# bentotten/radiation_ppo

Hardware: AMD Instinct MI355X
Metric: env steps/sec (whole node) at 4096 envs; PPO iters/sec at 1/2/4/8 GPUs (higher is better)
Workload: dtype f32 policy / f64+int32 env

## Files before the change

include/radsearch.h:

```cpp
#ifndef RADSEARCH_H
#define RADSEARCH_H

#include <stddef.h>
#include <stdint.h>

#ifdef __cplusplus
extern "C" {
#endif

#define RS_ABI_VERSION 4
#define RS_OBS_DIM 11
#define RS_NUM_ACTIONS 9
#define RS_MAX_AGENTS 8
#define RS_MAX_OBS 7

typedef void* rs_stream_t;
typedef struct rs_handle rs_handle;

enum {
    RS_OK = 0,
    RS_ERR_INVALID_ARG = 1,
    RS_ERR_HIP = 2,
    RS_ERR_WORKSPACE = 3,
    RS_ERR_UNSUPPORTED = 4
// ... 37 lines not shown
int rs_create(const rs_config* cfg, void* workspace, size_t workspace_bytes, rs_stream_t stream, rs_handle** out);
void rs_destroy(rs_handle* h);

int rs_state_field(rs_handle* h, const char* name, void** dev_ptr, int32_t* elem_bytes, int32_t* rows, int32_t* cols);

int rs_set_epoch_end(rs_handle* h, rs_stream_t stream);

int rs_reset(rs_handle* h, const uint8_t* mask, float* obs, float* reward, float* team, uint8_t* done,
             const rs_info* info, rs_stream_t stream);

int rs_refresh(rs_handle* h, const uint8_t* mask, const int32_t* src_xy, const int32_t* det_xy, const int32_t* intensity,
               const int32_t* bkg, const int32_t* num_obs, const int32_t* rects, float* obs, float* reward, float* team,
               uint8_t* done, const rs_info* info, rs_stream_t stream);

int rs_step(rs_handle* h, const int8_t* actions, float* obs, float* reward, float* team, uint8_t* done,
            const rs_info* info, rs_stream_t stream);

int rs_action_uniforms(rs_handle* h, float* u, rs_stream_t stream);

int rs_error_flags(rs_handle* h, rs_stream_t stream, uint32_t* flags_out);

int rs_gae(const float* rew, const float* val, const uint8_t* cut, const float* last_val, float* adv, float* ret,
           int32_t T, int32_t M, double gamma, double lam, rs_stream_t stream);

typedef struct rs_mlp_params {
    const float *w1, *b1, *w2, *b2, *w3, *b3;
} rs_mlp_params;

int rs_policy_forward(const rs_mlp_params* actor, const rs_mlp_params* critic, const float* x, int32_t M,
                      float* logits, float* value, rs_stream_t stream);

typedef struct rs_rollout_args {
    int32_t steps_per_epoch;
    int32_t steps_per_episode;
    float* obs;
    int64_t* act;
    float* logp;
    float* val;
    float* rew;
    float* last_val;
    uint8_t* cut;
    float* source_tar;
    float* cur_obs;
    double* w_count;
    double* w_mean;
    double* w_sq;
// ... 223 lines not shown
```

radiation_ppo_amd/_lib.py:

```python
import ctypes as C
import os

import torch

_PKG = os.path.dirname(os.path.abspath(__file__))
LIB_PATH = os.environ.get("RS_LIB_PATH") or os.path.join(_PKG, "lib", "librs_hip.so")

RS_OBS_DIM = 11
RS_MAX_AGENTS = 8
RS_MAX_OBS = 7

ENVERR_ZERO_DIST = 1
ENVERR_IDLE_STALL = 2
ENVERR_CORRECT_CAP = 4
ENVERR_BAD_ACTION = 8
ENVERR_NO_PATH = 16


class RsConfig(C.Structure):
    _fields_ = [
        ("num_envs", C.c_int32), ("num_agents", C.c_int32), ("obstruction_count", C.c_int32),
        ("enforce_grid_boundaries", C.c_int32), ("bbox", C.c_int32 * 4), ("observation_area", C.c_int32 * 2),
        ("falloff", C.c_int32), ("geom_group_size", C.c_int32), ("seed", C.c_uint32), ("env_id_base", C.c_uint32),
        ("coord_noise", C.c_int32), ("debug_spawn", C.c_int32),
# ... 53 lines not shown
                              C.c_void_p, C.c_void_p, C.c_void_p]),
    ("rs_adam_step", C.c_int, [C.POINTER(RsMlpParams), C.POINTER(RsMlpParams), C.c_void_p, C.c_void_p, C.c_void_p, C.c_void_p,
                               C.c_void_p, C.c_float, C.c_float, C.c_void_p]),
    ("rs_ppo_update_step", C.c_int, [C.POINTER(RsMlpParams), C.POINTER(RsMlpParams), C.POINTER(RsPpoBatch), C.c_void_p, C.c_void_p,
                                     C.c_void_p, C.c_void_p, C.c_void_p, C.c_void_p, C.c_float, C.c_float, C.c_void_p]),
    ("rs_maps_state_bytes", C.c_size_t, [C.c_int32, C.c_int32, C.c_int32, C.c_int32, C.c_int32]),
    ("rs_maps_create", C.c_int, [C.c_int32, C.c_int32, C.c_int32, C.c_int32, C.c_int32, C.c_double, C.c_void_p, C.c_void_p,
                                 C.c_size_t, C.c_void_p, C.POINTER(C.c_void_p)]),
    ("rs_maps_destroy", None, [C.c_void_p]),
    ("rs_maps_reset", C.c_int, [C.c_void_p, C.c_void_p, C.c_void_p]),
    ("rs_maps_update", C.c_int, [C.c_void_p, C.c_void_p, C.c_void_p, C.c_void_p, C.c_void_p, C.c_void_p]),
    ("rs_maps_stack", C.c_int, [C.c_void_p, C.c_void_p, C.c_void_p, C.c_void_p]),
    ("rs_maps_field", C.c_int, [C.c_void_p, C.c_char_p, C.POINTER(C.c_void_p), C.POINTER(C.c_int32), C.POINTER(C.c_int32),
                                C.POINTER(C.c_int32)]),
    ("rs_cnn_trunk_slab_row", C.c_int32, [C.c_int32]),
    ("rs_cnn_trunk_slab_rows", C.c_int32, [C.c_int64, C.c_int32]),
    ("rs_cnn_trunk_scratch_floats", C.c_int32, [C.c_int32]),
    ("rs_cnn_trunk_forward", C.c_int, [C.c_void_p, C.c_void_p, C.c_void_p, C.c_int32, C.c_int32, C.c_int64, C.c_void_p, C.c_void_p,
                                       C.c_void_p, C.c_void_p, C.c_void_p, C.c_void_p, C.c_void_p, C.c_void_p, C.c_void_p, C.c_void_p]),
    ("rs_cnn_trunk_backward", C.c_int, [C.c_void_p, C.c_void_p, C.c_void_p, C.c_int32, C.c_int32, C.c_int64, C.c_void_p, C.c_void_p,
                                        C.c_void_p, C.c_void_p, C.c_void_p, C.c_void_p, C.c_void_p, C.c_void_p]),
    ("rs_gae", C.c_int, [C.c_void_p, C.c_void_p, C.c_void_p, C.c_void_p, C.c_void_p, C.c_void_p, C.c_int32,
                         C.c_int32, C.c_double, C.c_double, C.c_void_p]),
    ("rs_pfgru_step", C.c_int, [C.c_void_p, C.c_void_p, C.c_void_p, C.c_void_p, C.c_void_p, C.c_void_p, C.c_void_p, C.c_void_p,
                                C.c_int32, C.c_double, C.c_void_p, C.c_int32, C.c_int32, C.c_void_p]),
    ("rs_pfgru_step_recorded", C.c_int, [C.c_void_p] * 7 + [C.c_int32, C.c_double, C.c_void_p, C.c_int32, C.c_int32, C.c_void_p]),
    ("rs_pfgru_pass", C.c_int, [C.c_void_p] * 7 + [C.c_double, C.c_void_p, C.c_void_p, C.c_int32, C.c_int32, C.c_void_p]),
    ("rs_pfgru_reset", C.c_int, [C.c_void_p, C.c_void_p, C.c_void_p, C.c_void_p, C.c_void_p, C.c_void_p, C.c_int32, C.c_int32,
                                 C.c_void_p]),
    ("rs_pfgru_sized_weight_floats", C.c_int32, [C.c_int32]),
    ("rs_pfgru_sized_step", C.c_int, [C.c_void_p] * 8 + [C.c_int32, C.c_double, C.c_void_p, C.c_int32, C.c_int32, C.c_int32, C.c_void_p]),
    ("rs_pfgru_sized_pass", C.c_int, [C.c_void_p] * 7 + [C.c_double, C.c_void_p, C.c_void_p, C.c_int32, C.c_int32, C.c_int32, C.c_void_p]),
    ("rs_pfgru_sized_step_recorded", C.c_int, [C.c_void_p] * 7 + [C.c_int32, C.c_double, C.c_void_p, C.c_int32, C.c_int32, C.c_int32,
                                                                    C.c_void_p]),
    ("rs_pfgru_sized_reset", C.c_int, [C.c_void_p] * 6 + [C.c_int32, C.c_int32, C.c_int32, C.c_void_p]),
    ("rs_pfgru_draws", C.c_int, [C.c_void_p, C.c_int32, C.c_int32, C.c_void_p, C.c_void_p, C.c_void_p, C.c_void_p]),
    ("rs_pfgru_train", C.c_int, [C.c_void_p] * 15 + [C.c_int32, C.c_int32, C.c_double, C.c_double, C.c_double, C.c_double, C.c_void_p]),
    ("rs_pfgru_train_keyed", C.c_int, [C.c_void_p] * 14 + [C.c_int32, C.c_int32, C.c_double, C.c_double, C.c_double, C.c_double, C.c_void_p]),
    ("rs_pfgru_sized_train_weight_floats", C.c_int32, [C.c_int32]),
    ("rs_pfgru_sized_train_grad_floats", C.c_int32, [C.c_int32]),
    ("rs_pfgru_sized_draws", C.c_int, [C.c_void_p, C.c_int32, C.c_int32, C.c_int32, C.c_void_p, C.c_void_p, C.c_void_p, C.c_void_p]),
    ("rs_pfgru_sized_train", C.c_int, [C.c_void_p] * 15 + [C.c_int32, C.c_int32, C.c_double, C.c_double, C.c_double, C.c_double, C.c_int32,
                                       C.c_void_p]),
    ("rs_rnn_policy_step", C.c_int, [C.c_void_p] * 10 + [C.c_int32, C.c_void_p]),
    ("rs_rnn_policy_step_rows", C.c_int, [C.c_void_p, C.c_void_p, C.c_int32, C.c_void_p, C.c_int32, C.c_void_p, C.c_void_p, C.c_int32, C.c_void_p,
                                          C.c_void_p, C.c_void_p, C.c_void_p, C.c_void_p, C.c_int32, C.c_void_p, C.c_int32, C.c_void_p]),
# ... 84 lines not shown
```

radiation_ppo_amd/csrc/rs_env.hip:

```cpp
#include <hip/hip_runtime.h>
#include <stdint.h>
#include <stdlib.h>
#include <string.h>
#include <new>

#include "../../include/radsearch.h"
#include "rs_device.hpp"
#include "rs_handle.hpp"

template <bool HAS_OBS>
__global__ void __launch_bounds__(64, (HAS_OBS ? 4 : 1)) rs_step_kernel(RsParams P, const int8_t* __restrict__ actions, float* obs, RsOut O) {
    extern __shared__ __align__(16) unsigned char smem[];
    int* lds_geo = reinterpret_cast<int*>(smem);
    float* tile = reinterpret_cast<float*>(smem + (HAS_OBS ? RS_MAX_VERT * RS_WAVE * 4 : 0));
    int* flags = reinterpret_cast<int*>(tile + RS_WAVE * rs_tile_stride(P.A));
    const int lane = threadIdx.x & 63;
    const int n = blockIdx.x * blockDim.x + threadIdx.x;
    const bool active = n < P.N;
    RsGeo g{lds_geo, 0, 0, 0};
    if (HAS_OBS) rs_load_geo(P, n, active, lds_geo, g);
    flags[lane] = active ? 1 : 0;
    __syncthreads();
    if (active) {
        RsOut o = O;
// ... 204 lines not shown
            const int t = tb - u;
            if (t >= t_lo) {
                const double r = (double)r8[u], v = (double)v8[u];
                if (c8[u]) {
                    const double lv = (double)l8[u];
                    v_next = lv;
                    r_acc = lv;
                    a_acc = 0.0;
                }
                const double delta = r + gamma * v_next - v;
                a_acc = delta + gl * a_acc;
                r_acc = r + gamma * r_acc;
                if (t <= t_hi) {
                    const size_t i = (size_t)t * M + m;
                    adv[i] = (float)a_acc;
                    ret[i] = (float)r_acc;
                }
                v_next = v;
            }
        }
#pragma unroll
        for (int u = 0; u < RS_GAE_U; ++u) { r8[u] = rn[u]; v8[u] = vn[u]; l8[u] = ln[u]; c8[u] = cn[u]; }
    }
}

static inline size_t align_up(size_t x, size_t a) { return (x + a - 1) / a * a; }

struct Carver {
    unsigned char* base; size_t off; rs_handle* h;
    template <typename T> T* take(const char* name, int rows, int cols) {
        off = align_up(off, 256);
        T* p = base ? reinterpret_cast<T*>(base + off) : nullptr;
        if (h) { h->fields[h->n_fields++] = rs_field{name, (void*)p, (int)sizeof(T), rows, cols}; }
        off += sizeof(T) * (size_t)rows * (size_t)cols;
        return p;
    }
};

static bool cfg_ok(const rs_config* c) {
    if (!c) return false;
    if (c->num_envs < 1 || c->num_agents < 1 || c->num_agents > RS_MAX_AGENTS) return false;
    if (c->obstruction_count < -1 || c->obstruction_count > RS_MAX_OBS) return false;
    if (c->geom_group_size < 1) return false;
    if (c->bbox[2] <= c->bbox[0] || c->bbox[3] <= c->bbox[1]) return false;
    if (c->bbox[2] > 16000 || c->bbox[3] > 16000 || c->bbox[0] < -16000 || c->bbox[1] < -16000) return false;
    if (c->observation_area[0] < 0 || c->observation_area[1] <= c->observation_area[0]) return false;
// ... 179 lines not shown
        hipStreamSynchronize(s) != hipSuccess) rc = RS_ERR_HIP;
    uint32_t acc = 0;
    if (rc == RS_OK) for (int i = 0; i < N; ++i) acc |= host[i];
    delete[] host;
    *flags_out = acc;
    return rc;
}

int rs_gae(const float* rew, const float* val, const uint8_t* cut, const float* last_val, float* adv, float* ret,
           int32_t T, int32_t M, double gamma, double lam, rs_stream_t stream) {
    if (!rew || !val || !cut || !last_val || !adv || !ret || T < 1 || M < 1) return RS_ERR_INVALID_ARG;
    hipStream_t s = static_cast<hipStream_t>(stream);
    const int col_waves = (M + 63) / 64;
    int chunks = (512 + col_waves - 1) / col_waves;
    chunks = chunks < 1 ? 1 : (chunks > 16 ? 16 : chunks);
    int chunk = (T + chunks - 1) / chunks;
    if (chunk < 32) chunk = 32;
    chunks = (T + chunk - 1) / chunk;
    hipLaunchKernelGGL(rs_gae_kernel, dim3(col_waves, chunks), dim3(64), 0, s, rew, val, cut, last_val, adv, ret, T, M,
                       gamma, gamma * lam, chunk);
    return hipGetLastError() == hipSuccess ? RS_OK : RS_ERR_HIP;
}

#ifdef RS_STEP_STAMPS
int rs_debug_step_stamps(unsigned long long* out, int clear) {
    if (hipDeviceSynchronize() != hipSuccess) return RS_ERR_HIP;
    if (out && hipMemcpyFromSymbol(out, HIP_SYMBOL(rs_step_stamp_table), sizeof(unsigned long long) * 16) != hipSuccess) return RS_ERR_HIP;
    if (clear) {
        unsigned long long z[16] = {0};
        if (hipMemcpyToSymbol(HIP_SYMBOL(rs_step_stamp_table), z, sizeof(z)) != hipSuccess) return RS_ERR_HIP;
    }
    return RS_OK;
}
#endif

}
```

radiation_ppo_amd/csrc/rs_ppo.hip:

```cpp
#include <hip/hip_runtime.h>
#include <stdint.h>
#include <stdlib.h>
#include <string.h>

#include "../../include/radsearch.h"
#include "rs_mlp.hpp"
#include "rs_handle.hpp"

static inline RsMlpParams to_dev(const rs_mlp_params* p) { return RsMlpParams{p->w1, p->b1, p->w2, p->b2, p->w3, p->b3}; }

__device__ __forceinline__ void rs_exchange_x(const float (&xo)[RS_IN_PAD], float (&xp)[RS_IN_PAD]) {
#pragma unroll
    for (int k = 0; k < RS_IN_PAD; ++k) xp[k] = __shfl_xor(xo[k], 32);
}

__global__ void __launch_bounds__(64) rs_policy_forward_kernel(RsMlpParams pa, RsMlpParams pc, const float* __restrict__ x, int M,
                                                               float* __restrict__ logits, float* __restrict__ value) {
    extern __shared__ __align__(16) float smem_f[];
    RsMlpLds<8> A; RsMlpLds<1> Cn;
    A.carve(smem_f);
    Cn.carve(smem_f + rs_mlp_lds_floats(8));
    A.fill(pa); Cn.fill(pc);
    __syncthreads();
    const int lane = threadIdx.x & 63;
// ... 260 lines not shown
    if (!actor || !critic || !grads || !m || !v || !state) return RS_ERR_INVALID_ARG;
    const RsParamSeg S = rs_param_seg(actor, critic);
    const int o = S.off[12];
    hipStream_t s = static_cast<hipStream_t>(stream);
    hipLaunchKernelGGL(rs_adam_apply_kernel, dim3((o + 255) / 256), dim3(256), 0, s, S, grads, m, v, stats, state, lr, kl_threshold);
    hipLaunchKernelGGL(rs_adam_commit_kernel, dim3(1), dim3(1), 0, s, stats, grads + o, state, kl_threshold);
    return hipGetLastError() == hipSuccess ? RS_OK : RS_ERR_HIP;
}

struct RsGradWs { float *pa, *pc; double *sa, *sc; int* snap; };

static RsGradWs rs_grad_ws(void* workspace) {
    const int slabs = RS_GRAD_BLOCKS;
    RsGradWs w;
    w.pa = static_cast<float*>(workspace);
    w.pc = w.pa + (size_t)slabs * rs_net_params(8);
    w.sa = reinterpret_cast<double*>((reinterpret_cast<uintptr_t>(w.pc + (size_t)slabs * rs_net_params(1)) + 255) & ~uintptr_t(255));
    w.sc = w.sa + (size_t)slabs * 5;
    w.snap = reinterpret_cast<int*>(w.sc + (size_t)slabs * 5);
    return w;
}

static int rs_launch_k7(const rs_mlp_params* actor, const rs_mlp_params* critic, const rs_ppo_batch* batch, const RsGradWs& w,
                        const int32_t* stop_flag, const rs_update_state* ust, hipStream_t s) {
    const size_t lds_a = sizeof(float) * (size_t)rs_grad2_lds_floats(8);
    const size_t lds_c = sizeof(float) * (size_t)rs_grad2_lds_floats(1);
    if (hipFuncSetAttribute(reinterpret_cast<const void*>(rs_ppo_grad2_kernel<8>), hipFuncAttributeMaxDynamicSharedMemorySize, (int)lds_a) != hipSuccess ||
        hipFuncSetAttribute(reinterpret_cast<const void*>(rs_ppo_grad2_kernel<1>), hipFuncAttributeMaxDynamicSharedMemorySize, (int)lds_c) != hipSuccess)
        return RS_ERR_HIP;
    int threads = 512;
#ifdef RS_K7_STAMPS
    if (const char* e = getenv("RS_K7_THREADS")) threads = atoi(e) == 256 ? 256 : 512;
#endif
    hipLaunchKernelGGL(rs_ppo_grad2_kernel<8>, dim3(RS_GRAD_BLOCKS), dim3(threads), lds_a, s, to_dev(actor), *batch, w.pa, w.sa, stop_flag,
                       (const rs_update_state*)nullptr, (int*)nullptr);
    hipLaunchKernelGGL(rs_ppo_grad2_kernel<1>, dim3(RS_GRAD_BLOCKS), dim3(threads), lds_c, s, to_dev(critic), *batch, w.pc, w.sc, stop_flag,
                       ust, ust ? w.snap : (int*)nullptr);
    return RS_OK;
}

int rs_ppo_grad(const rs_mlp_params* actor, const rs_mlp_params* critic, const rs_ppo_batch* batch, float* grads,
                double* stats, void* workspace, const int32_t* stop_flag, rs_stream_t stream) {
    if (!actor || !critic || !batch || !grads || !stats || !workspace || batch->M < 1) return RS_ERR_INVALID_ARG;
    if (reinterpret_cast<uintptr_t>(workspace) & 255u) return RS_ERR_WORKSPACE;
    hipStream_t s = static_cast<hipStream_t>(stream);
    const RsGradWs w = rs_grad_ws(workspace);
    if (const int rc = rs_launch_k7(actor, critic, batch, w, stop_flag, nullptr, s)) return rc;
    const int np = rs_net_params(8) + rs_net_params(1);
    hipLaunchKernelGGL(rs_ppo_reduce_kernel, dim3((np + 63) / 64), dim3(1024), 0, s, w.pa, w.pc, w.sa, w.sc, RS_GRAD_BLOCKS, grads, stats,
                       batch->alpha, batch->vf_coef, stop_flag);
    return hipGetLastError() == hipSuccess ? RS_OK : RS_ERR_HIP;
}

int rs_ppo_update_step(const rs_mlp_params* actor, const rs_mlp_params* critic, const rs_ppo_batch* batch, float* grads,
                       double* stats, void* workspace, float* m, float* v, rs_update_state* state, float lr, float kl_threshold,
                       rs_stream_t stream) {
    if (!actor || !critic || !batch || !grads || !stats || !workspace || !m || !v || !state || batch->M < 1) return RS_ERR_INVALID_ARG;
    if (reinterpret_cast<uintptr_t>(workspace) & 255u) return RS_ERR_WORKSPACE;
    hipStream_t s = static_cast<hipStream_t>(stream);
    const RsGradWs w = rs_grad_ws(workspace);
    if (const int rc = rs_launch_k7(actor, critic, batch, w, &state->stopped, state, s)) return rc;
    const int np = rs_net_params(8) + rs_net_params(1);
    hipLaunchKernelGGL(rs_ppo_tail_kernel, dim3((np + 63) / 64), dim3(1024), 0, s, w.pa, w.pc, w.sa, w.sc, RS_GRAD_BLOCKS, grads, stats,
                       batch->alpha, batch->vf_coef, rs_param_seg(actor, critic), m, v, state, w.snap, lr, kl_threshold);
    return hipGetLastError() == hipSuccess ? RS_OK : RS_ERR_HIP;
}

#ifdef RS_K7_STAMPS
int rs_debug_k7_stamps(unsigned long long* out, int clear) {
    if (hipDeviceSynchronize() != hipSuccess) return RS_ERR_HIP;
    if (out && hipMemcpyFromSymbol(out, HIP_SYMBOL(rs_k7_stamp_table), sizeof(unsigned long long) * 2 * RS_K7_NPH) != hipSuccess) return RS_ERR_HIP;
    if (clear) {
        unsigned long long z[2 * RS_K7_NPH] = {0};
        if (hipMemcpyToSymbol(HIP_SYMBOL(rs_k7_stamp_table), z, sizeof(z)) != hipSuccess) return RS_ERR_HIP;
    }
    return RS_OK;
}
#endif

int rs_policy_forward(const rs_mlp_params* actor, const rs_mlp_params* critic, const float* x, int32_t M,
                      float* logits, float* value, rs_stream_t stream) {
    if (!actor || !critic || !x || M < 1) return RS_ERR_INVALID_ARG;
    const int groups = (M + 63) / 64;
    const int grid = groups < 2048 ? groups : 2048;
// ... 8 lines not shown
```

radiation_ppo_amd/csrc/rs_ppo_grad2.hpp:

```cpp
#pragma once
#include "rs_mlp.hpp"

#define RS_T2 33

#ifdef RS_K7_STAMPS
#define RS_K7_NPH 16
__device__ unsigned long long rs_k7_stamp_table[2][RS_K7_NPH];
#define RS_STAMP_ENTRY const unsigned long long st_rt0 = __builtin_amdgcn_s_memrealtime(); const unsigned long long st_t0 = rs_k7_now();
#define RS_STAMP_DECL unsigned long long st_acc[RS_K7_NPH] = {0}; unsigned long long st_last = rs_k7_now(); st_acc[12] = st_last - st_t0;
#define RS_STAMP_EXIT(net) do { RS_STAMP(13); if ((threadIdx.x & 63) == 0) { st_acc[14] = __builtin_amdgcn_s_memrealtime() - st_rt0; \
                           for (int q = 0; q < RS_K7_NPH; ++q) atomicAdd(&rs_k7_stamp_table[net][q], st_acc[q]); } } while (0)
#define RS_STAMP(i) do { __builtin_amdgcn_sched_barrier(0); asm volatile("; RS_STAMP_MARK " #i); const unsigned long long t_ = rs_k7_now(); st_acc[i] += t_ - st_last; st_last = t_; \
                         __builtin_amdgcn_sched_barrier(0); } while (0)
__device__ __forceinline__ unsigned long long rs_k7_now() {
    unsigned long long t;
    asm volatile("s_memtime %0\n\ts_waitcnt lgkmcnt(0)" : "=s"(t) :: "memory");
    return t;
}
#else
#define RS_STAMP_ENTRY
#define RS_STAMP_DECL
#define RS_STAMP_EXIT(net)
#ifdef RS_K7_NO_PHASE_FENCE
#define RS_STAMP(i) do {} while (0)
#else
#define RS_STAMP(i) __builtin_amdgcn_sched_barrier(0)
#endif
#endif
#define RS_XRAW 400
#define RS_XSC 192
#define RS_G2_WAVE_FLOATS ((64 + 32) * RS_T2 + RS_XRAW + RS_XSC + 64)

__host__ __device__ constexpr int rs_grad2_lds_floats(int nout) {
    return ((rs_mlp_lds_floats(nout) + 3) & ~3) + 2 * 2 * 16 * 64 + 2 * 4 * 64 + 8 * RS_G2_WAVE_FLOATS;
}

__device__ __forceinline__ float rs_other_half(float x, int h) {
    const auto r = __builtin_amdgcn_permlane32_swap(__float_as_uint(x), __float_as_uint(x), false, false);
    return __uint_as_float(h ? r[0] : r[1]);
}

__device__ __forceinline__ void rs_stage32(float* T, const f32x16& v, int c, int h) {
#pragma unroll
    for (int r = 0; r < 16; ++r) T[rs_kappa(r, h) * RS_T2 + c] = v[r];
}

template <int NOUT>
__global__ void __launch_bounds__(512, 2) rs_ppo_grad2_kernel(RsMlpParams prm, rs_ppo_batch B, float* __restrict__ partial,
                                                              double* __restrict__ stat_partial, const int* __restrict__ stop,
                                                              const rs_update_state* __restrict__ ust, int* __restrict__ snap) {
    extern __shared__ __align__(16) float smem_f[];
    if (snap && blockIdx.x == 0 && threadIdx.x == 0) { snap[0] = ust->adam_step; snap[1] = ust->stopped; }
    if (stop && *stop) return;
    RS_STAMP_ENTRY
    RsMlpLds<NOUT> W;
    W.carve(smem_f);
    float* w2tf = smem_f + ((rs_mlp_lds_floats(NOUT) + 3) & ~3);
    float* w3tf = w2tf + 2 * 2 * 16 * 64;
    const int wid = __builtin_amdgcn_readfirstlane(threadIdx.x >> 6);
    const int lane = threadIdx.x & 63, h = lane >> 5, c = lane & 31;
    const int l15 = lane & 15, l4 = lane >> 4;
    float* Qt = w3tf + 2 * 4 * 64 + wid * RS_G2_WAVE_FLOATS;
    float* Pt = Qt + 64 * RS_T2;
    float* xraw = Pt + 32 * RS_T2;
    float* xsc = xraw + RS_XRAW;
    float* dbl = xsc + RS_XSC;
    float* w1b = W.w1f;
    for (int i = threadIdx.x; i < 2 * 6 * 64; i += blockDim.x) {
        const int l = i & 63, s = (i >> 6) % 6, it = i / (6 * 64);
        const int row = 32 * it + (l & 31), k = 2 * s + (l >> 5);
        w1b[i] = RS_TANH_PRESCALE * ((k < RS_IN) ? prm.w1[row * RS_IN + k] : prm.b1[row]);
    }
    for (int i = threadIdx.x; i < 2 * 2 * 16 * 64; i += blockDim.x) {
        const int ri = i & 3, l = (i >> 2) & 63, r4 = (i >> 8) & 3, kt = (i >> 10) & 1, it = i >> 11;
        const int r = 4 * r4 + ri;
        w2tf[i] = prm.w2[(32 * kt + rs_kappa(r, l >> 5)) * RS_HID + 32 * it + (l & 31)];
        W.w2f[i] = RS_TANH_PRESCALE * prm.w2[(32 * it + (l & 31)) * RS_HID + 32 * kt + rs_kappa(r, l >> 5)];
    }
    for (int i = threadIdx.x; i < 2 * 4 * 64; i += blockDim.x) {
        int l = i & 63, sq = (i >> 6) & 3, it = i >> 8;
        int o = 2 * sq + (l >> 5);
        w3tf[i] = (o < NOUT) ? prm.w3[o * RS_HID + 32 * it + (l & 31)] : 0.0f;
    }
    for (int i = threadIdx.x; i < 2 * NOUT * 32; i += blockDim.x) {
        const int q = i & 31, o = (i >> 5) % NOUT, hh = i / (32 * NOUT);
        W.w3h[i] = prm.w3[o * RS_HID + 32 * (q >> 4) + rs_kappa(q & 15, hh)];
    }
    for (int i = threadIdx.x; i < 64; i += blockDim.x) W.b2[i] = RS_TANH_PRESCALE * prm.b2[i];
    for (int i = threadIdx.x; i < NOUT; i += blockDim.x) W.b3[i] = prm.b3[i];
    dbl[lane] = 0.0f;
    __syncthreads();

    const int M = B.M;
    const int groups = (M + 31) / 32;
    const int wave_g = blockIdx.x * 8 + wid, n_waves = gridDim.x * 8;

    f32x16 acc2[2][2];
    f32x4 acc1[4], acc3[4];
#pragma unroll
    for (int a = 0; a < 2; ++a)
#pragma unroll
        for (int r = 0; r < 16; ++r) { acc2[a][0][r] = 0.f; acc2[a][1][r] = 0.f; }
#pragma unroll
    for (int a = 0; a < 4; ++a)
#pragma unroll
        for (int r = 0; r < 4; ++r) { acc1[a][r] = 0.f; acc3[a][r] = 0.f; }
    f32x4 accs;
#pragma unroll
    for (int r = 0; r < 4; ++r) accs[r] = 0.f;

    const int trips = (groups + n_waves - 1) / n_waves;
    const long x_last = (long)M * RS_IN - 1;
    auto dma_rows = [&](int g) {
        const char* gx = reinterpret_cast<const char*>(B.x + (long)g * (32 * RS_IN));
        const int lim = (int)(x_last - (long)g * (32 * RS_IN));
#pragma unroll
        for (int i = 0; i < 6; ++i) {
            const int o = min(i * 64 + lane, lim);
// ... 342 lines not shown
            for (int s = 0; s < 8; ++s) {
                float a0_n = 0.f, a1_n = 0.f;
                if (s + 1 < 8) {
                    a0_n = Pt[l15 * RS_T2 + 4 * (s + 1) + l4];
                    a1_n = Pt[(16 + l15) * RS_T2 + 4 * (s + 1) + l4];
                }
                acc1[2 * it + 0] = __builtin_amdgcn_mfma_f32_16x16x4f32(a0_c, xb[s], acc1[2 * it + 0], 0, 0, 0);
                acc1[2 * it + 1] = __builtin_amdgcn_mfma_f32_16x16x4f32(a1_c, xb[s], acc1[2 * it + 1], 0, 0, 0);
                a0_c = a0_n; a1_c = a1_n;
            }
        }
        rs_wave_sync();
        RS_STAMP(11);
    }
    constexpr int RS_REST = rs_net_params(NOUT) - 64 * 64;
    static_assert(8 * 64 * 64 <= rs_grad2_lds_floats(NOUT) && 8 * ((RS_REST + 1) & ~1) + 2 * 8 * 5 <= rs_grad2_lds_floats(NOUT),
                  "the epilogue's slabs must fit K7's LDS");
    int tid_e = threadIdx.x;
    asm volatile("" : "+v"(tid_e));
    const int lane_e = tid_e & 63, h_e = lane_e >> 5, c_e = lane_e & 31, l15_e = lane_e & 15, l4_e = lane_e >> 4;
    asm volatile("s_waitcnt vmcnt(0)" ::: "memory");
    const float db2v = dbl[lane_e];
    __syncthreads();
    float* outp = partial + (size_t)blockIdx.x * rs_net_params(NOUT);
    {
        float* g_w2 = smem_f + wid * (64 * 64);
#pragma unroll
        for (int it = 0; it < 2; ++it)
#pragma unroll
            for (int r = 0; r < 16; ++r) {
                const int row = 32 * it + rs_kappa(r, h_e);
                g_w2[row * 64 + c_e] = acc2[it][0][r];
                g_w2[row * 64 + 32 + c_e] = acc2[it][1][r];
            }
    }
    __syncthreads();
    for (int i = tid_e; i < 64 * 64; i += blockDim.x) {
        float v = 0.0f + smem_f[i];
#pragma unroll
        for (int wv = 1; wv < 8; ++wv) v += smem_f[wv * (64 * 64) + i];
        outp[64 * RS_IN + 64 + i] = v;
    }
    float db3r[NOUT];
#pragma unroll
    for (int o = 0; o < NOUT; ++o) db3r[o] = __shfl(accs[o & 3], 16 * (o >> 2));
    double sv[5];
    {
// ... 15 lines not shown
                if (l15_e < RS_IN) g_w1[row * RS_IN + l15_e] = acc1[u][q];
                if (l15_e == RS_IN) g_b1[row] = acc1[u][q];
                const int o = 4 * l4_e + q;
                if (o < NOUT) g_w3[o * 64 + 16 * u + l15_e] = acc3[u][q];
            }
        if (lane_e == 0) {
#pragma unroll
            for (int o = 0; o < NOUT; ++o) g_b3[o] = db3r[o];
#pragma unroll
            for (int q = 0; q < 5; ++q) sred[wid * 5 + q] = sv[q];
        }
    }
    __syncthreads();
    for (int i = tid_e; i < RS_REST; i += blockDim.x) {
        float v = 0.0f + smem_f[i];
#pragma unroll
        for (int wv = 1; wv < 8; ++wv) v += smem_f[wv * RS_RSTR + i];
        outp[i < 64 * RS_IN + 64 ? i : i + 64 * 64] = v;
    }
    if (tid_e < 5) {
        double v = 0.0 + sred[tid_e];
#pragma unroll
        for (int wv = 1; wv < 8; ++wv) v += sred[wv * 5 + tid_e];
        stat_partial[(size_t)blockIdx.x * 5 + tid_e] = v;
    }
    RS_STAMP_EXIT(NOUT == 8 ? 0 : 1);
}
```

radiation_ppo_amd/ppo.py:

```python
import ctypes as C
import os
from dataclasses import dataclass
from typing import Any, Dict, List, Optional

import torch
import torch.distributed as dist
import torch.nn as nn

from . import _lib
from .envs import RadSearchVec, gae as rs_gae_call


class FFActorCritic(nn.Module):

    def __init__(self, state_dim: int = 11, action_dim: int = 8, hidden: int = 64):
        super().__init__()
        self.actor = nn.Sequential(nn.Linear(state_dim, hidden), nn.Tanh(), nn.Linear(hidden, hidden), nn.Tanh(),
                                   nn.Linear(hidden, action_dim), nn.Softmax(dim=-1))
        self.critic = nn.Sequential(nn.Linear(state_dim, hidden), nn.Tanh(), nn.Linear(hidden, hidden), nn.Tanh(),
                                    nn.Linear(hidden, 1))

    def logits(self, x: torch.Tensor) -> torch.Tensor:
        for layer in list(self.actor)[:-1]:
            x = layer(x)
# ... 78 lines not shown
                                         torch.cuda.current_stream(self.grads.device).cuda_stream), "rs_adam_step")

    def read_state(self):
        st = self.state.cpu()
        i32 = st.view(torch.int32)
        return int(i32[2]), int(i32[1]), int(i32[0]), st[2:7].tolist()

    def __call__(self, X, act, adv, ret, logp_old, w, clip_ratio: float, alpha: float, vf_coef: float = 0.01,
                 use_stop_flag: bool = False):
        import ctypes as C
        for t in (X, adv, ret, logp_old, w):
            assert t.dtype == torch.float32 and t.is_contiguous()
        assert act.dtype == torch.int64 and act.is_contiguous()
        self.stats_from_bucket = False
        b = _lib.RsPpoBatch(X.data_ptr(), act.data_ptr(), adv.data_ptr(), ret.data_ptr(), logp_old.data_ptr(), w.data_ptr(),
                            X.shape[0], clip_ratio, alpha, vf_coef)
        pa, pc = mlp_params(self.ac.actor), mlp_params(self.ac.critic)
        with _lib.timed("rs_ppo_grad"):
            _lib.check(self.lib.rs_ppo_grad(C.byref(pa), C.byref(pc), C.byref(b), self.bucket.data_ptr(), self.stats.data_ptr(),
                                            self._ws_ptr, (self.state.data_ptr() + 4) if use_stop_flag else None,
                                            torch.cuda.current_stream(X.device).cuda_stream), "rs_ppo_grad")
        return self.stats, self.grads

    def step(self, X, act, adv, ret, logp_old, w, clip_ratio: float, alpha: float, vf_coef: float = 0.01, *, lr: float,
             kl_threshold: float):
        for t in (X, adv, ret, logp_old, w):
            assert t.dtype == torch.float32 and t.is_contiguous()
        assert act.dtype == torch.int64 and act.is_contiguous()
        self.stats_from_bucket = False
        b = _lib.RsPpoBatch(X.data_ptr(), act.data_ptr(), adv.data_ptr(), ret.data_ptr(), logp_old.data_ptr(), w.data_ptr(),
                            X.shape[0], clip_ratio, alpha, vf_coef)
        pa, pc = mlp_params(self.ac.actor), mlp_params(self.ac.critic)
        with _lib.timed("rs_ppo_grad"):
            _lib.check(self.lib.rs_ppo_update_step(C.byref(pa), C.byref(pc), C.byref(b), self.bucket.data_ptr(), self.stats.data_ptr(),
                                                   self._ws_ptr, self.m.data_ptr(), self.v.data_ptr(), self.state.data_ptr(), lr,
                                                   kl_threshold, torch.cuda.current_stream(X.device).cuda_stream), "rs_ppo_update_step")
        return self.stats, self.grads

    def allreduce(self) -> None:
        Collectives.all_reduce_sum(self.bucket)
        self.stats_from_bucket = True

    def assign_grads(self) -> None:
        for p, g in self.views:
            p.grad = g


class DeviceWelford:

    def __init__(self, shape, device, impl: Optional[str] = None):
        self.impl = impl or ("hip" if torch.device(device).type == "cuda" else "torch")
        assert self.impl in ("hip", "torch") and (self.impl == "torch" or torch.device(device).type == "cuda")
        self.count = torch.zeros(shape, dtype=torch.float64, device=device)
        self.mean = torch.zeros(shape, dtype=torch.float64, device=device)
        self.sq = torch.zeros(shape, dtype=torch.float64, device=device)
        self.std = torch.ones(shape, dtype=torch.float64, device=device)

    @staticmethod
    def _strided(t: torch.Tensor):
        if t.dim() == 2 and t.dtype == torch.float32 and t.stride(1) > 0 and t.stride(0) == t.shape[1] * t.stride(1):
# ... 246 lines not shown
                stats = torch.stack([(w * (logp_old - logp)).sum(), ent_m.detach(), (w * clipped.float()).sum(),
                                     val_loss.detach(), loss.detach()]).double()
            self.pi_optimizer.zero_grad(set_to_none=True)
            loss.backward()
            stats_h = host_read(reduce_grads_and_stats(self.agent.parameters(), stats))
            last = stats_h
            if stats_h[0] < thr:
                self.pi_optimizer.step()
            else:
                kl_reached = True
            kk += 1
        self.pi_scheduler.step()
        return UpdateResult(stop_iteration=kk, loss_policy=last[4], loss_critic=last[3], loss_predictor=0.0,
                            kl_divergence=last[0], Entropy=last[1], ClipFrac=last[2], LocLoss=0.0)

    def _update_agent_fused(self, X, act, adv, ret, logp_old, w) -> UpdateResult:
        if self._fused is None:
            self._fused = FusedPPOGrad(self.agent)
        f = self._fused
        lr = self.actor_learning_rate * (0.99 ** (self.epochs_done // 100))
        thr = 1.5 * self.target_kl
        f.begin_update()
        one_rank = _world() == 1 and not os.environ.get("RS_PPO_SPLIT_TAIL")
        for _ in range(self.train_pi_iters):
            if one_rank:
                f.step(X, act, adv, ret, logp_old, w, self.clip_ratio, self.alpha, lr=lr, kl_threshold=thr)
                continue
            stats, grads = f(X, act, adv, ret, logp_old, w, self.clip_ratio, self.alpha, use_stop_flag=True)
            if _world() > 1:
                f.allreduce()
            f.adam_step(lr, thr)
        kk, stopped, _, last = f.read_state()
        self.epochs_done += 1
        return UpdateResult(stop_iteration=kk, loss_policy=last[4], loss_critic=last[3], loss_predictor=0.0,
                            kl_divergence=last[0], Entropy=last[1], ClipFrac=last[2], LocLoss=0.0)

    def save(self, path: str) -> None:
        torch.save(self.agent.state_dict(), path)

    def load(self, path: str) -> None:
        self.agent.load_state_dict(torch.load(path, map_location=self.device, weights_only=True))

    def resume_state(self) -> Dict[str, Any]:
        st: Dict[str, Any] = dict(model=self.agent.state_dict(), epochs_done=self.epochs_done,
                                  pi_optimizer=self.pi_optimizer.state_dict(), pi_scheduler=self.pi_scheduler.state_dict())
        if self._fused is not None:
            f = self._fused
            st["fused"] = dict(m=f.m.clone(), v=f.v.clone(), adam_step=int(f.state_i32[0].item()))
        return st
# ... 245 lines not shown
        one = lambda t: t.double().sum().view(1)
        return dict(DoneCount=one(self.done_count), OutOfBound=one(self.oob_count), EpCount=self.ep_count.double().sum(),
                    EpLenSum=self.ep_len_sum.sum(), EpRetSum=one(self.ep_ret_sum), EpRetSqSum=one(self.ep_ret_sq),
                    EpRetMax=self.ep_ret_max.double().max().view(1), EpRetMin=self.ep_ret_min.double().min().view(1))

    def update(self) -> Dict[int, UpdateResult]:
        return ppo_update_from_buffer(self)

    _RESUME = ("cur_obs", "w_count", "w_mean", "w_sq", "w_std", "steps_in_ep", "ep_ret")

    def resume_state(self) -> Dict[str, Any]:
        if not self.started:
            self.start()
        return dict(env=self.env.snapshot(), **{k: getattr(self, k).clone() for k in self._RESUME})

    def load_resume_state(self, st: Dict[str, Any]) -> None:
        if not self.started:
            self.start()
        self.env.restore(st["env"])
        for k in self._RESUME:
            getattr(self, k).copy_(st[k])


def ppo_update_from_buffer(col) -> Dict[int, UpdateResult]:
    buf = col.buf
    n_total = col.N * _world()
    w = (buf.episode_weights() / n_total).reshape(-1)
    out = {}
    for a, ag in col.agents.items():
        adv = normalize_advantages(buf.adv[:, :, a]).reshape(-1)
        X = buf.obs[:, :, a].reshape(-1, buf.obs.shape[-1])
        out[a] = ag.update_agent(X, buf.act[:, :, a].reshape(-1), adv, buf.ret[:, :, a].reshape(-1),
                                 buf.logp[:, :, a].reshape(-1), w)
    return out
```

Measured before the change: 39.65 million.

## Fuse PPO update prep into HIP kernels, pair actor/critic grad launch, cache bindings

Adds HIP kernels that compute per-step episode weights and advantage normalization in three launches, replacing a series of torch ops on the single-rank, single-agent path. It also merges the actor and critic gradient kernels into one paired launch that splits the grid between them. Finally it binds the ctypes batch and parameter structs once per update rather than on every PPO iteration. Together these aim to cut kernel launch count and Python/host overhead in the update phase, at the cost of a new code path whose float normalization and weight arithmetic may differ slightly from the torch version.

```diff
diff --git a/include/radsearch.h b/include/radsearch.h
--- a/include/radsearch.h
+++ b/include/radsearch.h
@@ -83,6 +83,10 @@
 
 int rs_gae(const float* rew, const float* val, const uint8_t* cut, const float* last_val, float* adv, float* ret,
            int32_t T, int32_t M, double gamma, double lam, rs_stream_t stream);
+
+size_t rs_ppo_prepare_workspace_bytes(int32_t N);
+int rs_ppo_prepare(const uint8_t* cut, const float* adv, float* w, float* adv_n, float* mean_std, void* workspace, int32_t T, int32_t N,
+                   int32_t n_total, rs_stream_t stream);
 
 typedef struct rs_mlp_params {
     const float *w1, *b1, *w2, *b2, *w3, *b3;
diff --git a/radiation_ppo_amd/_lib.py b/radiation_ppo_amd/_lib.py
--- a/radiation_ppo_amd/_lib.py
+++ b/radiation_ppo_amd/_lib.py
@@ -99,6 +99,8 @@
                                         C.c_void_p, C.c_void_p, C.c_void_p, C.c_void_p, C.c_void_p, C.c_void_p]),
     ("rs_gae", C.c_int, [C.c_void_p, C.c_void_p, C.c_void_p, C.c_void_p, C.c_void_p, C.c_void_p, C.c_int32,
                          C.c_int32, C.c_double, C.c_double, C.c_void_p]),
+    ("rs_ppo_prepare_workspace_bytes", C.c_size_t, [C.c_int32]),
+    ("rs_ppo_prepare", C.c_int, [C.c_void_p] * 6 + [C.c_int32, C.c_int32, C.c_int32, C.c_void_p]),
     ("rs_pfgru_step", C.c_int, [C.c_void_p, C.c_void_p, C.c_void_p, C.c_void_p, C.c_void_p, C.c_void_p, C.c_void_p, C.c_void_p,
                                 C.c_int32, C.c_double, C.c_void_p, C.c_int32, C.c_int32, C.c_void_p]),
     ("rs_pfgru_step_recorded", C.c_int, [C.c_void_p] * 7 + [C.c_int32, C.c_double, C.c_void_p, C.c_int32, C.c_int32, C.c_void_p]),
diff --git a/radiation_ppo_amd/csrc/rs_env.hip b/radiation_ppo_amd/csrc/rs_env.hip
--- a/radiation_ppo_amd/csrc/rs_env.hip
+++ b/radiation_ppo_amd/csrc/rs_env.hip
@@ -250,6 +250,111 @@
 #pragma unroll
         for (int u = 0; u < RS_GAE_U; ++u) { r8[u] = rn[u]; v8[u] = vn[u]; l8[u] = ln[u]; c8[u] = cn[u]; }
     }
+}
+
+#define RS_PREP_U 16
+#define RS_PREP_BLOCKS 256
+#define RS_PREP_THREADS 256
+
+__global__ void __launch_bounds__(64) rs_ppo_prepare_cols_kernel(const uint8_t* __restrict__ cut, const float* __restrict__ adv,
+                                                                 float* __restrict__ w, double* __restrict__ col_sums, int T, int N,
+                                                                 float inv_n_total) {
+    __shared__ double lane_sum[64];
+    const int n = blockIdx.x * 64 + threadIdx.x;
+    const bool live = n < N;
+    const int nn = live ? n : N - 1;
+    int pos = 0, n_ep = 1;
+    double s = 0.0;
+    for (int tb = 0; tb < T; tb += RS_PREP_U) {
+        uint8_t c[RS_PREP_U];
+        float a[RS_PREP_U];
+#pragma unroll
+        for (int u = 0; u < RS_PREP_U; ++u) {
+            const size_t i = (size_t)min(tb + u, T - 1) * N + nn;
+            c[u] = cut[i]; a[u] = adv[i];
+        }
+#pragma unroll
+        for (int u = 0; u < RS_PREP_U; ++u) {
+            const int t = tb + u;
+            if (t < T) {
+                s += (double)a[u];
+                if (live) w[(size_t)t * N + n] = __int_as_float(pos);
+                if (c[u]) { pos = 0; n_ep += (t < T - 1) ? 1 : 0; } else ++pos;
+            }
+        }
+    }
+    const float n_ep_f = (float)n_ep;
+    int left = 0;
+    for (int tb = T - 1; tb >= 0; tb -= RS_PREP_U) {
+        uint8_t c[RS_PREP_U];
+        int ps[RS_PREP_U];
+#pragma unroll
+        for (int u = 0; u < RS_PREP_U; ++u) {
+            const size_t i = (size_t)max(tb - u, 0) * N + nn;
+            c[u] = cut[i]; ps[u] = __float_as_int(w[i]);
+        }
+#pragma unroll
+        for (int u = 0; u < RS_PREP_U; ++u) {
+            const int t = tb - u;
+            if (t >= 0) {
+                left = (c[u] || t == T - 1) ? 0 : left + 1;
+                const float len = (float)(ps[u] + left + 1);
+                if (live) w[(size_t)t * N + n] = (1.0f / (n_ep_f * len)) * inv_n_total;
+            }
+        }
+    }
+    lane_sum[threadIdx.x] = live ? s : 0.0;
+    __syncthreads();
+    if (threadIdx.x == 0) {
+        double v = 0.0;
+        for (int i = 0; i < 64; ++i) v += lane_sum[i];
+        col_sums[blockIdx.x] = v;
+    }
+}
+
+__device__ __forceinline__ double rs_prep_sum(const double* __restrict__ p, int n, double* red) {
+    double v = 0.0;
+    for (int i = threadIdx.x; i < n; i += RS_PREP_THREADS) v += p[i];
+    __syncthreads();
+    red[threadIdx.x] = v;
+    __syncthreads();
+    if (threadIdx.x == 0) {
+        double t = 0.0;
+        for (int i = 0; i < RS_PREP_THREADS; ++i) t += red[i];
+        red[RS_PREP_THREADS] = t;
+    }
+    __syncthreads();
+    return red[RS_PREP_THREADS];
+}
+
+__global__ void __launch_bounds__(RS_PREP_THREADS) rs_ppo_prepare_sq_kernel(const float* __restrict__ adv, const double* __restrict__ col_sums,
+                                                                            int n_col_sums, double* __restrict__ sq_sums, size_t n) {
+    __shared__ double red[RS_PREP_THREADS + 1];
+    const float mean = (float)(rs_prep_sum(col_sums, n_col_sums, red) / (double)n);
+    double v = 0.0;
+    for (size_t i = (size_t)blockIdx.x * RS_PREP_THREADS + threadIdx.x; i < n; i += (size_t)RS_PREP_BLOCKS * RS_PREP_THREADS) {
+        const float d = adv[i] - mean;
+        v += (double)(d * d);
+    }
+    __syncthreads();
+    red[threadIdx.x] = v;
+    __syncthreads();
+    if (threadIdx.x == 0) {
+        double t = 0.0;
+        for (int i = 0; i < RS_PREP_THREADS; ++i) t += red[i];
+        sq_sums[blockIdx.x] = t;
+    }
+}
+
+__global__ void __launch_bounds__(RS_PREP_THREADS) rs_ppo_prepare_norm_kernel(const float* __restrict__ adv, const double* __restrict__ col_sums,
+                                                                              int n_col_sums, const double* __restrict__ sq_sums,
+                                                                              float* __restrict__ adv_n, float* __restrict__ mean_std, size_t n) {
+    __shared__ double red[RS_PREP_THREADS + 1];
+    const float mean = (float)(rs_prep_sum(col_sums, n_col_sums, red) / (double)n);
+    const float sd = (float)sqrt(rs_prep_sum(sq_sums, RS_PREP_BLOCKS, red) / (double)n);
+    for (size_t i = (size_t)blockIdx.x * RS_PREP_THREADS + threadIdx.x; i < n; i += (size_t)RS_PREP_BLOCKS * RS_PREP_THREADS)
+        adv_n[i] = (adv[i] - mean) / sd;
+    if (blockIdx.x == 0 && threadIdx.x == 0) { mean_std[0] = mean; mean_std[1] = sd; }
 }
 
 static inline size_t align_up(size_t x, size_t a) { return (x + a - 1) / a * a; }
@@ -475,6 +580,28 @@
     return hipGetLastError() == hipSuccess ? RS_OK : RS_ERR_HIP;
 }
 
+size_t rs_ppo_prepare_workspace_bytes(int32_t N) {
+    if (N < 1) return 0;
+    return sizeof(double) * ((size_t)(N + 63) / 64 + RS_PREP_BLOCKS);
+}
+
+int rs_ppo_prepare(const uint8_t* cut, const float* adv, float* w, float* adv_n, float* mean_std, void* workspace, int32_t T, int32_t N,
+                   int32_t n_total, rs_stream_t stream) {
+    if (!cut || !adv || !w || !adv_n || !mean_std || !workspace || T < 1 || N < 1 || n_total < 1) return RS_ERR_INVALID_ARG;
+    if (reinterpret_cast<uintptr_t>(workspace) & 7u) return RS_ERR_WORKSPACE;
+    hipStream_t s = static_cast<hipStream_t>(stream);
+    const int col_groups = (N + 63) / 64;
+    double* col_sums = static_cast<double*>(workspace);
+    double* sq_sums = col_sums + col_groups;
+    const size_t n = (size_t)T * (size_t)N;
+    const float inv_n_total = (float)(1.0 / (double)n_total);
+    hipLaunchKernelGGL(rs_ppo_prepare_cols_kernel, dim3(col_groups), dim3(64), 0, s, cut, adv, w, col_sums, T, N, inv_n_total);
+    hipLaunchKernelGGL(rs_ppo_prepare_sq_kernel, dim3(RS_PREP_BLOCKS), dim3(RS_PREP_THREADS), 0, s, adv, col_sums, col_groups, sq_sums, n);
+    hipLaunchKernelGGL(rs_ppo_prepare_norm_kernel, dim3(RS_PREP_BLOCKS), dim3(RS_PREP_THREADS), 0, s, adv, col_sums, col_groups, sq_sums, adv_n,
+                       mean_std, n);
+    return hipGetLastError() == hipSuccess ? RS_OK : RS_ERR_HIP;
+}
+
 #ifdef RS_STEP_STAMPS
 int rs_debug_step_stamps(unsigned long long* out, int clear) {
     if (hipDeviceSynchronize() != hipSuccess) return RS_ERR_HIP;
diff --git a/radiation_ppo_amd/csrc/rs_ppo.hip b/radiation_ppo_amd/csrc/rs_ppo.hip
--- a/radiation_ppo_amd/csrc/rs_ppo.hip
+++ b/radiation_ppo_amd/csrc/rs_ppo.hip
@@ -306,16 +306,25 @@
 }
 
 static int rs_launch_k7(const rs_mlp_params* actor, const rs_mlp_params* critic, const rs_ppo_batch* batch, const RsGradWs& w,
-                        const int32_t* stop_flag, const rs_update_state* ust, hipStream_t s) {
+                        const int32_t* stop_flag, const rs_update_state* ust, hipStream_t s, bool pair = false) {
     const size_t lds_a = sizeof(float) * (size_t)rs_grad2_lds_floats(8);
     const size_t lds_c = sizeof(float) * (size_t)rs_grad2_lds_floats(1);
-    if (hipFuncSetAttribute(reinterpret_cast<const void*>(rs_ppo_grad2_kernel<8>), hipFuncAttributeMaxDynamicSharedMemorySize, (int)lds_a) != hipSuccess ||
-        hipFuncSetAttribute(reinterpret_cast<const void*>(rs_ppo_grad2_kernel<1>), hipFuncAttributeMaxDynamicSharedMemorySize, (int)lds_c) != hipSuccess)
+    const size_t lds_p = lds_a > lds_c ? lds_a : lds_c;
+    if (pair) {
+        if (hipFuncSetAttribute(reinterpret_cast<const void*>(rs_ppo_grad2_pair_kernel), hipFuncAttributeMaxDynamicSharedMemorySize, (int)lds_p) != hipSuccess)
+            return RS_ERR_HIP;
+    } else if (hipFuncSetAttribute(reinterpret_cast<const void*>(rs_ppo_grad2_kernel<8>), hipFuncAttributeMaxDynamicSharedMemorySize, (int)lds_a) != hipSuccess ||
+               hipFuncSetAttribute(reinterpret_cast<const void*>(rs_ppo_grad2_kernel<1>), hipFuncAttributeMaxDynamicSharedMemorySize, (int)lds_c) != hipSuccess)
         return RS_ERR_HIP;
     int threads = 512;
 #ifdef RS_K7_STAMPS
     if (const char* e = getenv("RS_K7_THREADS")) threads = atoi(e) == 256 ? 256 : 512;
 #endif
+    if (pair) {
+        hipLaunchKernelGGL(rs_ppo_grad2_pair_kernel, dim3(2 * RS_GRAD_BLOCKS), dim3(threads), lds_p, s, to_dev(actor), to_dev(critic), *batch,
+                           w.pa, w.pc, w.sa, w.sc, stop_flag, ust, ust ? w.snap : (int*)nullptr);
+        return RS_OK;
+    }
     hipLaunchKernelGGL(rs_ppo_grad2_kernel<8>, dim3(RS_GRAD_BLOCKS), dim3(threads), lds_a, s, to_dev(actor), *batch, w.pa, w.sa, stop_flag,
                        (const rs_update_state*)nullptr, (int*)nullptr);
     hipLaunchKernelGGL(rs_ppo_grad2_kernel<1>, dim3(RS_GRAD_BLOCKS), dim3(threads), lds_c, s, to_dev(critic), *batch, w.pc, w.sc, stop_flag,
@@ -343,7 +352,8 @@
     if (reinterpret_cast<uintptr_t>(workspace) & 255u) return RS_ERR_WORKSPACE;
     hipStream_t s = static_cast<hipStream_t>(stream);
     const RsGradWs w = rs_grad_ws(workspace);
-    if (const int rc = rs_launch_k7(actor, critic, batch, w, &state->stopped, state, s)) return rc;
+    const char* split = getenv("RS_PPO_SPLIT_GRAD");
+    if (const int rc = rs_launch_k7(actor, critic, batch, w, &state->stopped, state, s, !(split && *split && *split != '0'))) return rc;
     const int np = rs_net_params(8) + rs_net_params(1);
     hipLaunchKernelGGL(rs_ppo_tail_kernel, dim3((np + 63) / 64), dim3(1024), 0, s, w.pa, w.pc, w.sa, w.sc, RS_GRAD_BLOCKS, grads, stats,
                        batch->alpha, batch->vf_coef, rs_param_seg(actor, critic), m, v, state, w.snap, lr, kl_threshold);
diff --git a/radiation_ppo_amd/csrc/rs_ppo_grad2.hpp b/radiation_ppo_amd/csrc/rs_ppo_grad2.hpp
--- a/radiation_ppo_amd/csrc/rs_ppo_grad2.hpp
+++ b/radiation_ppo_amd/csrc/rs_ppo_grad2.hpp
@@ -46,11 +46,12 @@
 }
 
 template <int NOUT>
-__global__ void __launch_bounds__(512, 2) rs_ppo_grad2_kernel(RsMlpParams prm, rs_ppo_batch B, float* __restrict__ partial,
-                                                              double* __restrict__ stat_partial, const int* __restrict__ stop,
-                                                              const rs_update_state* __restrict__ ust, int* __restrict__ snap) {
+__device__ __forceinline__ void rs_ppo_grad2_body(const RsMlpParams prm, const rs_ppo_batch B, float* partial,
+                                                  double* stat_partial, const int* stop,
+                                                  const rs_update_state* ust, int* snap,
+                                                  const int bid, const int nblocks) {
     extern __shared__ __align__(16) float smem_f[];
-    if (snap && blockIdx.x == 0 && threadIdx.x == 0) { snap[0] = ust->adam_step; snap[1] = ust->stopped; }
+    if (snap && bid == 0 && threadIdx.x == 0) { snap[0] = ust->adam_step; snap[1] = ust->stopped; }
     if (stop && *stop) return;
     RS_STAMP_ENTRY
     RsMlpLds<NOUT> W;
@@ -93,7 +94,7 @@
 
     const int M = B.M;
     const int groups = (M + 31) / 32;
-    const int wave_g = blockIdx.x * 8 + wid, n_waves = gridDim.x * 8;
+    const int wave_g = bid * 8 + wid, n_waves = nblocks * 8;
 
     f32x16 acc2[2][2];
     f32x4 acc1[4], acc3[4];
@@ -482,7 +483,7 @@
     asm volatile("s_waitcnt vmcnt(0)" ::: "memory");
     const float db2v = dbl[lane_e];
     __syncthreads();
-    float* outp = partial + (size_t)blockIdx.x * rs_net_params(NOUT);
+    float* outp = partial + (size_t)bid * rs_net_params(NOUT);
     {
         float* g_w2 = smem_f + wid * (64 * 64);
 #pragma unroll
@@ -544,7 +545,23 @@
         double v = 0.0 + sred[tid_e];
 #pragma unroll
         for (int wv = 1; wv < 8; ++wv) v += sred[wv * 5 + tid_e];
-        stat_partial[(size_t)blockIdx.x * 5 + tid_e] = v;
+        stat_partial[(size_t)bid * 5 + tid_e] = v;
     }
     RS_STAMP_EXIT(NOUT == 8 ? 0 : 1);
 }
+
+template <int NOUT>
+__global__ void __launch_bounds__(512, 2) rs_ppo_grad2_kernel(RsMlpParams prm, rs_ppo_batch B, float* __restrict__ partial,
+                                                              double* __restrict__ stat_partial, const int* __restrict__ stop,
+                                                              const rs_update_state* __restrict__ ust, int* __restrict__ snap) {
+    rs_ppo_grad2_body<NOUT>(prm, B, partial, stat_partial, stop, ust, snap, blockIdx.x, gridDim.x);
+}
+
+__global__ void __launch_bounds__(512, 2) rs_ppo_grad2_pair_kernel(RsMlpParams pa, RsMlpParams pc, rs_ppo_batch B, float* __restrict__ partial_a,
+                                                                   float* __restrict__ partial_c, double* __restrict__ stat_a,
+                                                                   double* __restrict__ stat_c, const int* __restrict__ stop,
+                                                                   const rs_update_state* __restrict__ ust, int* __restrict__ snap) {
+    const int G = gridDim.x >> 1;
+    if ((int)blockIdx.x < G) rs_ppo_grad2_body<8>(pa, B, partial_a, stat_a, stop, nullptr, nullptr, blockIdx.x, G);
+    else rs_ppo_grad2_body<1>(pc, B, partial_c, stat_c, stop, ust, snap, blockIdx.x - G, G);
+}
diff --git a/radiation_ppo_amd/ppo.py b/radiation_ppo_amd/ppo.py
--- a/radiation_ppo_amd/ppo.py
+++ b/radiation_ppo_amd/ppo.py
@@ -124,20 +124,30 @@
                                             torch.cuda.current_stream(X.device).cuda_stream), "rs_ppo_grad")
         return self.stats, self.grads
 
-    def step(self, X, act, adv, ret, logp_old, w, clip_ratio: float, alpha: float, vf_coef: float = 0.01, *, lr: float,
-             kl_threshold: float):
+    def bind(self, X, act, adv, ret, logp_old, w, clip_ratio: float, alpha: float, vf_coef: float = 0.01) -> None:
+        import ctypes as C
         for t in (X, adv, ret, logp_old, w):
             assert t.dtype == torch.float32 and t.is_contiguous()
         assert act.dtype == torch.int64 and act.is_contiguous()
-        self.stats_from_bucket = False
         b = _lib.RsPpoBatch(X.data_ptr(), act.data_ptr(), adv.data_ptr(), ret.data_ptr(), logp_old.data_ptr(), w.data_ptr(),
                             X.shape[0], clip_ratio, alpha, vf_coef)
         pa, pc = mlp_params(self.ac.actor), mlp_params(self.ac.critic)
+        self._bound = (b, pa, pc, (X, act, adv, ret, logp_old, w))
+        self._bound_args = (C.byref(pa), C.byref(pc), C.byref(b), self.bucket.data_ptr(), self.stats.data_ptr(), self._ws_ptr,
+                            self.m.data_ptr(), self.v.data_ptr(), self.state.data_ptr())
+        self._bound_dev = X.device
+
+    def step_bound(self, lr: float, kl_threshold: float):
+        self.stats_from_bucket = False
         with _lib.timed("rs_ppo_grad"):
-            _lib.check(self.lib.rs_ppo_update_step(C.byref(pa), C.byref(pc), C.byref(b), self.bucket.data_ptr(), self.stats.data_ptr(),
-                                                   self._ws_ptr, self.m.data_ptr(), self.v.data_ptr(), self.state.data_ptr(), lr,
-                                                   kl_threshold, torch.cuda.current_stream(X.device).cuda_stream), "rs_ppo_update_step")
+            _lib.check(self.lib.rs_ppo_update_step(*self._bound_args, lr, kl_threshold,
+                                                   torch.cuda.current_stream(self._bound_dev).cuda_stream), "rs_ppo_update_step")
         return self.stats, self.grads
+
+    def step(self, X, act, adv, ret, logp_old, w, clip_ratio: float, alpha: float, vf_coef: float = 0.01, *, lr: float,
+             kl_threshold: float):
+        self.bind(X, act, adv, ret, logp_old, w, clip_ratio, alpha, vf_coef)
+        return self.step_bound(lr, kl_threshold)
 
     def allreduce(self) -> None:
         Collectives.all_reduce_sum(self.bucket)
@@ -430,9 +440,11 @@
         thr = 1.5 * self.target_kl
         f.begin_update()
         one_rank = _world() == 1 and not os.environ.get("RS_PPO_SPLIT_TAIL")
+        if one_rank:
+            f.bind(X, act, adv, ret, logp_old, w, self.clip_ratio, self.alpha)
         for _ in range(self.train_pi_iters):
             if one_rank:
-                f.step(X, act, adv, ret, logp_old, w, self.clip_ratio, self.alpha, lr=lr, kl_threshold=thr)
+                f.step_bound(lr, thr)
                 continue
             stats, grads = f(X, act, adv, ret, logp_old, w, self.clip_ratio, self.alpha, use_stop_flag=True)
             if _world() > 1:
@@ -724,11 +736,33 @@
             getattr(self, k).copy_(st[k])
 
 
+def prepare_update_hip(col):
+    buf = col.buf
+    lib = _lib.load()
+    p = getattr(col, "_prep", None)
+    if p is None:
+        dev = buf.adv.device
+        p = col._prep = dict(w=torch.empty(buf.T * buf.N, dtype=torch.float32, device=dev),
+                             adv_n=torch.empty(buf.T * buf.N, dtype=torch.float32, device=dev),
+                             mean_std=torch.empty(2, dtype=torch.float32, device=dev),
+                             ws=torch.empty((lib.rs_ppo_prepare_workspace_bytes(buf.N) + 7) // 8, dtype=torch.float64, device=dev))
+    _lib.check(lib.rs_ppo_prepare(buf.cut.data_ptr(), buf.adv.data_ptr(), p["w"].data_ptr(), p["adv_n"].data_ptr(), p["mean_std"].data_ptr(),
+                                  p["ws"].data_ptr(), buf.T, buf.N, col.N, torch.cuda.current_stream(buf.adv.device).cuda_stream),
+               "rs_ppo_prepare")
+    return p["w"], p["adv_n"]
+
+
 def ppo_update_from_buffer(col) -> Dict[int, UpdateResult]:
     buf = col.buf
     n_total = col.N * _world()
+    out = {}
+    if _world() == 1 and buf.adv.is_cuda and buf.A == 1 and len(col.agents) == 1 and buf.N == col.N:
+        w, adv = prepare_update_hip(col)
+        (a, ag), = col.agents.items()
+        X = buf.obs[:, :, a].reshape(-1, buf.obs.shape[-1])
+        out[a] = ag.update_agent(X, buf.act[:, :, a].reshape(-1), adv, buf.ret[:, :, a].reshape(-1), buf.logp[:, :, a].reshape(-1), w)
+        return out
     w = (buf.episode_weights() / n_total).reshape(-1)
-    out = {}
     for a, ag in col.agents.items():
         adv = normalize_advantages(buf.adv[:, :, a]).reshape(-1)
         X = buf.obs[:, :, a].reshape(-1, buf.obs.shape[-1])
```

After: 40.07 million, median of 6. 1.1% higher.
